# Fantom-foundation/go-txflow

Measured on AMD Instinct MI355X. Metric: verified+tallied TxVotes/sec, higher is better.
Workload: dtype u32

## Files before the change

go-txflow_amd/csrc/ed25519_dev.h:

```cpp
#pragma once
#include "fe.h"
#include "sc.h"
#include "sha2.h"
#include "ge.h"

namespace txv {

template <int W>
struct Tab {
  static constexpr int kPositions = (256 + W - 1) / W;
  static constexpr int kEntries = (1 << (W - 1)) + 1;
  static constexpr bool kLongTop = false;
  static constexpr int kTopEntries = kEntries;
  static constexpr size_t kWords = (size_t)kPositions * kEntries * kEntryWords;
  static constexpr uint64_t kBuildLanes = (uint64_t)kPositions * ((kEntries - 1) / 8);
};

template <>
struct Tab<21> {
  static constexpr int kPositions = 12;
  static constexpr int kEntries = (1 << 20) + 1;
  static constexpr bool kLongTop = true;
  static constexpr int kTopEntries = (1 << 21) + 9;
  static constexpr size_t kWords = ((size_t)(kPositions - 1) * kEntries + kTopEntries) * kEntryWords;
// ... 53 lines not shown
  const uint32_t pad_word = total >> 3, pad_shift = 56u - 8u * (total & 7u);
  const uint32_t last = 16u * nblk - 1u;
  uint64_t nx[16];
#pragma unroll
  for (int t = 0; t < 16; ++t) nx[t] = t < pre_words ? pre[t] : msg_word(m, (uint32_t)(t - pre_words));
  for (uint32_t b = 0; b < nblk; ++b) {
    uint64_t w[16];
#pragma unroll
    for (int t = 0; t < 16; ++t) {
      const uint32_t gw = 16u * b + (uint32_t)t;
      uint64_t v = nx[t];
      if (gw == pad_word) v |= 0x80ull << pad_shift;
      if (gw == last) v = (uint64_t)total * 8u;
      w[t] = v;
    }
    if (b + 1 < nblk) {
#pragma unroll
      for (int t = 0; t < 16; ++t) nx[t] = msg_word(m, 16u * (b + 1) + (uint32_t)t - (uint32_t)pre_words);
    }
    sha512_block(st, w);
  }
#pragma unroll
  for (int k = 0; k < 8; ++k) {
    digest_le[2 * k] = bswap32((uint32_t)(st[k] >> 32));
    digest_le[2 * k + 1] = bswap32((uint32_t)st[k]);
  }
}

TXV_HD void sha512_prefixed2(uint32_t dig0[16], const uint64_t* pre0, const MsgView& m0, uint32_t dig1[16],
                             const uint64_t* pre1, const MsgView& m1, int pre_words) {
  uint64_t st0[8], st1[8];
  sha512_init(st0);
  sha512_init(st1);
  const uint32_t tot0 = 8u * (uint32_t)pre_words + m0.len, tot1 = 8u * (uint32_t)pre_words + m1.len;
  const uint32_t nb0 = sha512_nblocks(tot0), nb1 = sha512_nblocks(tot1), nb = nb0 > nb1 ? nb0 : nb1;
  const uint32_t pw0 = tot0 >> 3, ps0 = 56u - 8u * (tot0 & 7u), last0 = 16u * nb0 - 1u;
  const uint32_t pw1 = tot1 >> 3, ps1 = 56u - 8u * (tot1 & 7u), last1 = 16u * nb1 - 1u;
  for (uint32_t b = 0; b < nb; ++b) {
    uint64_t w0[16], w1[16];
#pragma unroll
    for (int t = 0; t < 16; ++t) {
      const uint32_t gw = 16u * b + (uint32_t)t;
      uint64_t v0 = (b == 0 && t < pre_words) ? pre0[t] : msg_word(m0, gw - (uint32_t)pre_words);
      uint64_t v1 = (b == 0 && t < pre_words) ? pre1[t] : msg_word(m1, gw - (uint32_t)pre_words);
      if (gw == pw0) v0 |= 0x80ull << ps0;
      if (gw == last0) v0 = (uint64_t)tot0 * 8u;
      if (gw == pw1) v1 |= 0x80ull << ps1;
      if (gw == last1) v1 = (uint64_t)tot1 * 8u;
      w0[t] = v0;
      w1[t] = v1;
    }
    uint64_t s0[8], s1[8];
#pragma unroll
    for (int k = 0; k < 8; ++k) { s0[k] = st0[k]; s1[k] = st1[k]; }
    sha512_block2(s0, w0, s1, w1);
#pragma unroll
    for (int k = 0; k < 8; ++k) {
      if (b < nb0) st0[k] = s0[k];
      if (b < nb1) st1[k] = s1[k];
    }
  }
#pragma unroll
  for (int k = 0; k < 8; ++k) {
    dig0[2 * k] = bswap32((uint32_t)(st0[k] >> 32));
    dig0[2 * k + 1] = bswap32((uint32_t)st0[k]);
    dig1[2 * k] = bswap32((uint32_t)(st1[k] >> 32));
    dig1[2 * k + 1] = bswap32((uint32_t)st1[k]);
  }
}

template <int W, typename Ptr>
TXV_HD void load_entry_w(Ptr tab, int pos, int idx, bool neg, fe10& qp, fe10& qm, fe10& qd) {
#if defined(TXV_EXP_L2_TABLES)
  const size_t base = (size_t)(1 + (idx & 1)) * kEntryWords;
#else
  const size_t base = (size_t)(uint32_t)(pos * Tab<W>::kEntries + idx) * kEntryWords;
#endif
#ifndef TXV_ENTRY_LOADS
#define TXV_ENTRY_LOADS 1
#endif
#if TXV_ENTRY_LOADS == 2
  const uint4* e4 = reinterpret_cast<const uint4*>(&tab[base]);
  uint32_t w[32];
#pragma unroll
  for (int j = 0; j < 8; ++j) {
    const uint4 x = e4[j];
    w[4 * j] = x.x; w[4 * j + 1] = x.y; w[4 * j + 2] = x.z; w[4 * j + 3] = x.w;
  }
#pragma unroll
  for (int i = 0; i < 10; ++i) {
    qd.v[i] = w[kEntryQd + i];
    qm.v[i] = neg ? w[i] : w[kEntryQm + i];
    qp.v[i] = neg ? w[kEntryQm + i] : w[i];
  }
#else
  const uint32_t op = neg ? kEntryQm : 0u, om = neg ? 0u : kEntryQm;
  const uint2* d2 = reinterpret_cast<const uint2*>(&tab[base + kEntryQd]);
  const uint2 d0 = d2[0];
  const uint4 d1 = reinterpret_cast<const uint4*>(d2 + 1)[0], d3 = reinterpret_cast<const uint4*>(d2 + 1)[1];
  const uint4* m4 = reinterpret_cast<const uint4*>(&tab[base + om]);
  const uint4 m0 = m4[0], m1 = m4[1];
  const uint2 m2 = reinterpret_cast<const uint2*>(m4 + 2)[0];
  const uint4* p4 = reinterpret_cast<const uint4*>(&tab[base + op]);
  const uint4 p0 = p4[0], p1 = p4[1];
  const uint2 p2 = reinterpret_cast<const uint2*>(p4 + 2)[0];
  qp.v[0] = p0.x; qp.v[1] = p0.y; qp.v[2] = p0.z; qp.v[3] = p0.w;
  qp.v[4] = p1.x; qp.v[5] = p1.y; qp.v[6] = p1.z; qp.v[7] = p1.w; qp.v[8] = p2.x; qp.v[9] = p2.y;
  qm.v[0] = m0.x; qm.v[1] = m0.y; qm.v[2] = m0.z; qm.v[3] = m0.w;
  qm.v[4] = m1.x; qm.v[5] = m1.y; qm.v[6] = m1.z; qm.v[7] = m1.w; qm.v[8] = m2.x; qm.v[9] = m2.y;
  qd.v[0] = d0.x; qd.v[1] = d0.y; qd.v[2] = d1.x; qd.v[3] = d1.y;
  qd.v[4] = d1.z; qd.v[5] = d1.w; qd.v[6] = d3.x; qd.v[7] = d3.y; qd.v[8] = d3.z; qd.v[9] = d3.w;
#endif
}

template <int W>
TXV_HD int next_digit(uint32_t s[8], uint32_t& carry) {
  constexpr uint32_t mask = (1u << W) - 1u, half = 1u << (W - 1);
  const uint32_t d = (s[0] & mask) + carry;
  carry = (d + half) >> W;
#pragma unroll
  for (int i = 0; i < 7; ++i) s[i] = (s[i] >> W) | (s[i + 1] << (32 - W));
  s[7] >>= W;
  return (int)d - (int)(carry << W);
}

template <int W>
TXV_HD int table_digit(uint32_t s[8], uint32_t& carry, int pos) {
  if constexpr (Tab<W>::kLongTop) {
    if (pos == Tab<W>::kPositions - 1) return (int)(s[0] + carry);
  }
  return next_digit<W>(s, carry);
}

template <int W, int N>
TXV_HD void signed_digits(const uint32_t s[8], int d[N]) {
  constexpr uint32_t mask = (1u << W) - 1u, half = 1u << (W - 1);
  uint32_t carry = 0;
#pragma unroll
  for (int i = 0; i < N; ++i) {
    const int b = W * i, w = b >> 5, o = b & 31;
    uint32_t win = s[w] >> o;
    if (o + W > 32 && w + 1 < 8) win |= s[w + 1] << (32 - o);
    if (Tab<W>::kLongTop && i == Tab<W>::kPositions - 1) {
      static_assert(!Tab<W>::kLongTop || W * (Tab<W>::kPositions - 1) % 32 + 22 <= 32, "top digit in one word");
      d[i] = (int)(win + carry);
      break;
    }
    const uint32_t dd = (win & mask) + carry;
    carry = (dd + half) >> W;
    d[i] = (int)dd - (int)(carry << W);
  }
}

template <int WB, int WA, typename PtrB, typename PtrA>
TXV_HD ge_ext double_scalarmult_w2(PtrB tb, PtrA ta, const uint32_t s_in[8], const uint32_t k_in[8], bool use_a) {
  static_assert(WB >= WA, "B window must be at least the A window");
  uint32_t s[8], k[8], cs = 0, ck = 0;
#pragma unroll
  for (int i = 0; i < 8; ++i) { s[i] = s_in[i]; k[i] = k_in[i]; }
  fe10 qp, qm, qd;
  ge10_ext P;
  {
    const int ds = next_digit<WB>(s, cs);
    load_entry_w<WB>(tb, 0, ds < 0 ? -ds : ds, ds < 0, qp, qm, qd);
    P = ge10_from_entry(qp, qm);
  }
  for (int pos = 0; pos < Tab<WA>::kPositions; ++pos) {
    if (pos > 0 && pos < Tab<WB>::kPositions) {
      const int ds = next_digit<WB>(s, cs);
      load_entry_w<WB>(tb, pos, ds < 0 ? -ds : ds, ds < 0, qp, qm, qd);
      P = ge10_madd(P, qp, qm, qd, ds < 0);
    }
    if (use_a) {
      const int dk = table_digit<WA>(k, ck, pos);
      load_entry_w<WA>(ta, pos, dk < 0 ? -dk : dk, dk > 0, qp, qm, qd);
      P = ge10_madd(P, qp, qm, qd, dk > 0);
    }
  }
  ge_ext R;
  R.X = fe_from_fe10(P.X);
  R.Y = fe_from_fe10(P.Y);
  R.Z = fe_from_fe10(P.Z);
  R.T = fe_zero();
  return R;
}
template <int W, typename PtrB, typename PtrA>
TXV_HD ge_ext double_scalarmult_w(PtrB tb, PtrA ta, const uint32_t s_in[8], const uint32_t k_in[8], bool use_a) {
  return double_scalarmult_w2<W, W>(tb, ta, s_in, k_in, use_a);
}

template <typename PtrB, typename PtrA>
TXV_HD ge_ext double_scalarmult_fixed(PtrB tb, PtrA ta, const uint32_t s[8], const uint32_t k[8], bool use_a) {
  return double_scalarmult_w<4>(tb, ta, s, k, use_a);
}

TXV_HD ge_ext ge_mul_small(const ge_ext& P, uint32_t m) {
  ge_ext R = P;
  int top = 31 - __builtin_clz(m);
  for (int b = top - 1; b >= 0; --b) {
    R = ge_dbl(R);
    if ((m >> b) & 1u) R = ge_add(R, P);
  }
  return R;
}

TXV_HD void base_point_words(uint32_t w[8]) {
  const uint32_t b[8] = {0x66666658u, 0x66666666u, 0x66666666u, 0x66666666u,
                         0x66666666u, 0x66666666u, 0x66666666u, 0x66666666u};
#pragma unroll
  for (int i = 0; i < 8; ++i) w[i] = b[i];
}

}
```

go-txflow_amd/csrc/fe10.h:

```cpp
#pragma once
#include "fe.h"

namespace txv {

struct fe10 { uint32_t v[10]; };

#define TXV_W10(i) (((i) & 1) ? 25 : 26)
#define TXV_M10(i) (((i) & 1) ? 0x1ffffffu : 0x3ffffffu)

TXV_HD uint32_t fe10_2p(int i) { return i == 0 ? 0x7ffffdau : ((i & 1) ? 0x3fffffeu : 0x7fffffeu); }

TXV_HD fe10 fe10_zero() { fe10 r; for (int i = 0; i < 10; ++i) r.v[i] = 0; return r; }
TXV_HD fe10 fe10_one() { fe10 r = fe10_zero(); r.v[0] = 1; return r; }

TXV_HD fe10 fe10_add(const fe10& a, const fe10& b) {
  fe10 r;
#pragma unroll
  for (int i = 0; i < 10; ++i) r.v[i] = a.v[i] + b.v[i];
  return r;
}
TXV_HD fe10 fe10_sub(const fe10& a, const fe10& b) {
  fe10 r;
#pragma unroll
  for (int i = 0; i < 10; ++i) r.v[i] = (a.v[i] + fe10_2p(i)) - b.v[i];
  return r;
}
TXV_HD fe10 fe10_cneg(const fe10& a, bool neg) {
  const uint32_t m = neg ? 0xffffffffu : 0u;
  fe10 r;
#pragma unroll
  for (int i = 0; i < 10; ++i) r.v[i] = (a.v[i] ^ m) + (m & (fe10_2p(i) + 1u));
  return r;
}

TXV_HD fe10 fe10_carry(const fe10& a) {
  fe10 r = a;
  uint32_t c = 0;
#pragma unroll
  for (int i = 0; i < 10; ++i) {
    const uint32_t t = r.v[i] + c;
    c = t >> TXV_W10(i);
    r.v[i] = t & TXV_M10(i);
  }
  const uint32_t t = r.v[0] + 19u * c;
  r.v[0] = t & 0x3ffffffu;
  r.v[1] += t >> 26;
  return r;
}

#ifndef TXV_FE10_MUL
#define TXV_FE10_MUL 1
#endif
TXV_HD uint64_t fe10_col(uint64_t cin, const uint32_t a[10], const uint32_t b[10]) {
#if defined(__HIP_DEVICE_COMPILE__) && TXV_FE10_MUL == 2
  uint64_t x, y, cc;
  asm("v_mad_u64_u32 %0, %2, %3, %13, %23\n\t"
      "v_mad_u64_u32 %1, %2, %4, %14, 0\n\t"
      "v_mad_u64_u32 %0, %2, %5, %15, %0\n\t"
      "v_mad_u64_u32 %1, %2, %6, %16, %1\n\t"
      "v_mad_u64_u32 %0, %2, %7, %17, %0\n\t"
      "v_mad_u64_u32 %1, %2, %8, %18, %1\n\t"
      "v_mad_u64_u32 %0, %2, %9, %19, %0\n\t"
      "v_mad_u64_u32 %1, %2, %10, %20, %1\n\t"
      "v_mad_u64_u32 %0, %2, %11, %21, %0\n\t"
      "v_mad_u64_u32 %1, %2, %12, %22, %1\n\t"
      "v_lshl_add_u64 %0, %0, 0, %1"
      : "=&v"(x), "=&v"(y), "=&s"(cc)
      : "v"(a[0]), "v"(a[1]), "v"(a[2]), "v"(a[3]), "v"(a[4]), "v"(a[5]), "v"(a[6]), "v"(a[7]), "v"(a[8]), "v"(a[9]),
        "v"(b[0]), "v"(b[1]), "v"(b[2]), "v"(b[3]), "v"(b[4]), "v"(b[5]), "v"(b[6]), "v"(b[7]), "v"(b[8]), "v"(b[9]),
        "v"(cin));
  return x;
#elif defined(__HIP_DEVICE_COMPILE__) && TXV_FE10_MUL == 1
  uint64_t acc, cc;
  asm("v_mad_u64_u32 %0, %1, %2, %12, %22\n\t"
      "v_mad_u64_u32 %0, %1, %3, %13, %0\n\t"
      "v_mad_u64_u32 %0, %1, %4, %14, %0\n\t"
      "v_mad_u64_u32 %0, %1, %5, %15, %0\n\t"
      "v_mad_u64_u32 %0, %1, %6, %16, %0\n\t"
      "v_mad_u64_u32 %0, %1, %7, %17, %0\n\t"
      "v_mad_u64_u32 %0, %1, %8, %18, %0\n\t"
      "v_mad_u64_u32 %0, %1, %9, %19, %0\n\t"
      "v_mad_u64_u32 %0, %1, %10, %20, %0\n\t"
      "v_mad_u64_u32 %0, %1, %11, %21, %0"
      : "=&v"(acc), "=&s"(cc)
      : "v"(a[0]), "v"(a[1]), "v"(a[2]), "v"(a[3]), "v"(a[4]), "v"(a[5]), "v"(a[6]), "v"(a[7]), "v"(a[8]), "v"(a[9]),
        "v"(b[0]), "v"(b[1]), "v"(b[2]), "v"(b[3]), "v"(b[4]), "v"(b[5]), "v"(b[6]), "v"(b[7]), "v"(b[8]), "v"(b[9]),
        "v"(cin));
  return acc;
#else
  uint64_t acc = cin;
  for (int i = 0; i < 10; ++i) acc += (uint64_t)a[i] * b[i];
  return acc;
#endif
}

TXV_HD fe10 fe10_mul(const fe10& f, const fe10& g) {
  uint32_t g19[10], f2[10];
#pragma unroll
  for (int j = 1; j < 10; ++j) g19[j] = 19u * g.v[j];
#pragma unroll
  for (int i = 0; i < 10; ++i) f2[i] = (i & 1) ? f.v[i] + f.v[i] : f.v[i];
  g19[0] = 0;
  fe10 h;
  uint64_t acc = 0;
#pragma unroll
  for (int k = 0; k < 10; ++k) {
    uint32_t a[10], b[10];
#pragma unroll
    for (int i = 0; i < 10; ++i) {
      a[i] = ((i & 1) && !(k & 1)) ? f2[i] : f.v[i];
      b[i] = i <= k ? g.v[k - i] : g19[k + 10 - i];
    }
    acc = fe10_col(acc, a, b);
    h.v[k] = (uint32_t)acc & TXV_M10(k);
    acc >>= TXV_W10(k);
  }
  const uint64_t t = (uint64_t)(uint32_t)acc * 19u + h.v[0] + ((uint64_t)((uint32_t)(acc >> 32) * 19u) << 32);
  h.v[0] = (uint32_t)t & 0x3ffffffu;
  h.v[1] += (uint32_t)(t >> 26);
  return h;
}

TXV_HD void fe10_col2(uint64_t c1, const uint32_t a[10], const uint32_t b[10], uint64_t c2, const uint32_t x[10],
                      const uint32_t y[10], uint64_t& o1, uint64_t& o2) {
#if defined(__HIP_DEVICE_COMPILE__)
  uint64_t p, q, cc;
  asm("v_mad_u64_u32 %0, %2, %3, %13, %43\n\t"
      "v_mad_u64_u32 %1, %2, %23, %33, %44\n\t"
      "v_mad_u64_u32 %0, %2, %4, %14, %0\n\t"
      "v_mad_u64_u32 %1, %2, %24, %34, %1\n\t"
      "v_mad_u64_u32 %0, %2, %5, %15, %0\n\t"
      "v_mad_u64_u32 %1, %2, %25, %35, %1\n\t"
      "v_mad_u64_u32 %0, %2, %6, %16, %0\n\t"
      "v_mad_u64_u32 %1, %2, %26, %36, %1\n\t"
      "v_mad_u64_u32 %0, %2, %7, %17, %0\n\t"
      "v_mad_u64_u32 %1, %2, %27, %37, %1\n\t"
      "v_mad_u64_u32 %0, %2, %8, %18, %0\n\t"
      "v_mad_u64_u32 %1, %2, %28, %38, %1\n\t"
      "v_mad_u64_u32 %0, %2, %9, %19, %0\n\t"
      "v_mad_u64_u32 %1, %2, %29, %39, %1\n\t"
      "v_mad_u64_u32 %0, %2, %10, %20, %0\n\t"
      "v_mad_u64_u32 %1, %2, %30, %40, %1\n\t"
      "v_mad_u64_u32 %0, %2, %11, %21, %0\n\t"
      "v_mad_u64_u32 %1, %2, %31, %41, %1\n\t"
      "v_mad_u64_u32 %0, %2, %12, %22, %0\n\t"
      "v_mad_u64_u32 %1, %2, %32, %42, %1"
      : "=&v"(p), "=&v"(q), "=&s"(cc)
      : "v"(a[0]), "v"(a[1]), "v"(a[2]), "v"(a[3]), "v"(a[4]), "v"(a[5]), "v"(a[6]), "v"(a[7]), "v"(a[8]), "v"(a[9]),
        "v"(b[0]), "v"(b[1]), "v"(b[2]), "v"(b[3]), "v"(b[4]), "v"(b[5]), "v"(b[6]), "v"(b[7]), "v"(b[8]), "v"(b[9]),
        "v"(x[0]), "v"(x[1]), "v"(x[2]), "v"(x[3]), "v"(x[4]), "v"(x[5]), "v"(x[6]), "v"(x[7]), "v"(x[8]), "v"(x[9]),
        "v"(y[0]), "v"(y[1]), "v"(y[2]), "v"(y[3]), "v"(y[4]), "v"(y[5]), "v"(y[6]), "v"(y[7]), "v"(y[8]), "v"(y[9]),
        "v"(c1), "v"(c2));
  o1 = p;
  o2 = q;
#else
  uint64_t p = c1, q = c2;
  for (int i = 0; i < 10; ++i) {
    p += (uint64_t)a[i] * b[i];
    q += (uint64_t)x[i] * y[i];
  }
  o1 = p;
  o2 = q;
#endif
}

TXV_HD void fe10_mul2(const fe10& f1, const fe10& g1, const fe10& f2, const fe10& g2, fe10& h1, fe10& h2) {
  uint32_t g19a[10], f2a[10], g19b[10], f2b[10];
#pragma unroll
  for (int j = 1; j < 10; ++j) {
    g19a[j] = 19u * g1.v[j];
    g19b[j] = 19u * g2.v[j];
  }
#pragma unroll
  for (int i = 0; i < 10; ++i) {
    f2a[i] = (i & 1) ? f1.v[i] + f1.v[i] : f1.v[i];
    f2b[i] = (i & 1) ? f2.v[i] + f2.v[i] : f2.v[i];
  }
  g19a[0] = g19b[0] = 0;
  fe10 r1, r2;
  uint64_t acc1 = 0, acc2 = 0;
#pragma unroll
  for (int k = 0; k < 10; ++k) {
    uint32_t a[10], b[10], x[10], y[10];
#pragma unroll
    for (int i = 0; i < 10; ++i) {
      const bool dbl = (i & 1) && !(k & 1);
      a[i] = dbl ? f2a[i] : f1.v[i];
      x[i] = dbl ? f2b[i] : f2.v[i];
      b[i] = i <= k ? g1.v[k - i] : g19a[k + 10 - i];
      y[i] = i <= k ? g2.v[k - i] : g19b[k + 10 - i];
    }
    fe10_col2(acc1, a, b, acc2, x, y, acc1, acc2);
    r1.v[k] = (uint32_t)acc1 & TXV_M10(k);
    r2.v[k] = (uint32_t)acc2 & TXV_M10(k);
    acc1 >>= TXV_W10(k);
    acc2 >>= TXV_W10(k);
  }
  const uint64_t t1 = (uint64_t)(uint32_t)acc1 * 19u + r1.v[0] + ((uint64_t)((uint32_t)(acc1 >> 32) * 19u) << 32);
  const uint64_t t2 = (uint64_t)(uint32_t)acc2 * 19u + r2.v[0] + ((uint64_t)((uint32_t)(acc2 >> 32) * 19u) << 32);
  r1.v[0] = (uint32_t)t1 & 0x3ffffffu;
  r1.v[1] += (uint32_t)(t1 >> 26);
  r2.v[0] = (uint32_t)t2 & 0x3ffffffu;
  r2.v[1] += (uint32_t)(t2 >> 26);
  h1 = r1;
  h2 = r2;
}

TXV_HD fe10 fe10_strict(const fe10& a) {
  fe10 r = fe10_carry(a);
  uint32_t c = 0;
#pragma unroll
  for (int i = 1; i < 10; ++i) {
    const uint32_t t = r.v[i] + c;
    c = t >> TXV_W10(i);
    r.v[i] = t & TXV_M10(i);
  }
  const uint32_t t = r.v[0] + 19u * c;
  r.v[0] = t & 0x3ffffffu;
  r.v[1] += t >> 26;
  return r;
}

TXV_HD fe10 fe10_from_fe(const fe& a) {
  fe10 r;
  const uint32_t top = a.v[7] >> 31;
  int bit = 0;
#pragma unroll
  for (int i = 0; i < 10; ++i) {
    const int w = bit >> 5, s = bit & 31;
    uint32_t x = a.v[w] >> s;
    if (s + TXV_W10(i) > 32 && w < 7) x |= a.v[w + 1] << (32 - s);
    r.v[i] = x & TXV_M10(i);
    bit += TXV_W10(i);
  }
  r.v[0] += 19u * top;
  return r;
}

TXV_HD fe fe_from_fe10(const fe10& a) {
  const fe10 s = fe10_strict(a);
  fe r;
#pragma unroll
  for (int w = 0; w < 8; ++w) r.v[w] = 0;
  int bit = 0;
#pragma unroll
  for (int i = 0; i < 10; ++i) {
    const int w = bit >> 5, sh = bit & 31;
    r.v[w] |= s.v[i] << sh;
    if (sh + TXV_W10(i) > 32 && w < 7) r.v[w + 1] |= s.v[i] >> (32 - sh);
    bit += TXV_W10(i);
  }
  return r;
}

}
```

go-txflow_amd/csrc/kernels_verify.hip:

```cpp
#include <algorithm>
#include <cstdlib>

#include "ed25519_dev.h"
#include "fe_inv_var.h"
#include "txv_device.h"

using namespace txv;

#ifndef TXV_K1A_PREFETCH
#define TXV_K1A_PREFETCH 0
#endif

#ifndef TXV_INV_VAR
#define TXV_INV_VAR 1
#endif
__device__ __forceinline__ fe verify_invert(const fe& z) {
#if TXV_INV_VAR
  return fe_invert_var(z);
#else
  return fe_invert(z);
#endif
}

template <int W>
// ... 204 lines not shown
    }
    if (!act[0] && !act[1]) continue;
    ge_ext R;
    for (int h = 0; h < 2; ++h) {
      const uint32_t i = vi[h];
      if (act[h]) {
        const uint32_t v = a.val[i];
        uint32_t s[8], k[8];
#pragma unroll
        for (int j = 0; j < 8; ++j) { s[j] = a.sig[(size_t)(8 + j) * a.n_pad + i]; k[j] = a.kbuf[(size_t)j * a.n_pad + i]; }
        R = double_scalarmult_w<W>(a.btable, a.atables + (size_t)tab_slot(a, v) * Tab<W>::kWords, s, k, true);
      } else {
        R = ge_identity();
      }
      if (h == 0) {
#pragma unroll
        for (int j = 0; j < 8; ++j) {
          park[j][threadIdx.x] = R.X.v[j];
          park[8 + j][threadIdx.x] = R.Y.v[j];
          park[16 + j][threadIdx.x] = R.Z.v[j];
        }
      }
    }
    fe X0, Y0, Z0;
#pragma unroll
    for (int j = 0; j < 8; ++j) {
      X0.v[j] = park[j][threadIdx.x];
      Y0.v[j] = park[8 + j][threadIdx.x];
      Z0.v[j] = park[16 + j][threadIdx.x];
    }
    const fe inv = verify_invert(fe_mul(Z0, R.Z));
    uint32_t enc[8];
#pragma unroll
    for (int h = 0; h < 2; ++h) {
      if (h == 0) ge_encode_zinv(enc, X0, Y0, fe_mul(inv, R.Z));
      else ge_encode_zinv(enc, R.X, R.Y, fe_mul(inv, Z0));
      if (act[h]) {
        uint32_t diff = 0;
#pragma unroll
        for (int j = 0; j < 8; ++j) diff |= enc[j] ^ a.sig[(size_t)j * a.n_pad + vi[h]];
        a.ok_out[vi[h]] = diff == 0;
      }
    }
  }
}

#ifndef TXV_K1B_PREFETCH
#define TXV_K1B_PREFETCH 1
#endif

#ifndef TXV_K1B_NO_GATHER
#define TXV_K1B_NO_GATHER 0
#endif
__device__ __forceinline__ void entries_to_lds(const uint32_t* base, uint32_t e_l, uint4* buf) {
  if (TXV_K1B_NO_GATHER) return;
  const int lane = threadIdx.x & 63;
  uint32_t e[8];
#pragma unroll
  for (int i = 0; i < 8; ++i) e[i] = (uint32_t)__builtin_amdgcn_ds_bpermute((8 * i + (lane >> 3)) << 2, (int)e_l);
  TXV_SCHED_FENCE();
#pragma unroll
  for (int i = 0; i < 8; ++i) {
    const uint32_t piece = (uint32_t)((lane & 7) + 8 * i + (lane >> 3)) & 7u;
    const uint32_t* g = base + (size_t)e[i] * kEntryWords + piece * 4u;
    __builtin_amdgcn_global_load_lds((const __attribute__((address_space(1))) void*)g,
                                     (__attribute__((address_space(3))) void*)(buf + 64 * i), 16, 0, 0);
  }
}

__device__ __forceinline__ const uint4* entry_piece(const uint4* buf, int j) {
  const int e = threadIdx.x & 63;
  return buf + 64 * (e >> 3) + 8 * (e & 7) + ((j - e) & 7);
}

__device__ __forceinline__ fe10 entry_field_lds(const uint4* buf, bool neg, int role) {
  fe10 r;
  if (role == 2) {
    const uint2 d0 = reinterpret_cast<const uint2*>(entry_piece(buf, 5))[1];
    const uint4 d1 = *entry_piece(buf, 6), d2 = *entry_piece(buf, 7);
    r.v[0] = d0.x; r.v[1] = d0.y; r.v[2] = d1.x; r.v[3] = d1.y;
    r.v[4] = d1.z; r.v[5] = d1.w; r.v[6] = d2.x; r.v[7] = d2.y; r.v[8] = d2.z; r.v[9] = d2.w;
    return r;
  }
  const int j0 = (neg != (role == 1)) ? 3 : 0;
  const uint4 p0 = *entry_piece(buf, j0), p1 = *entry_piece(buf, j0 + 1);
  const uint2 p2 = *reinterpret_cast<const uint2*>(entry_piece(buf, j0 + 2));
  r.v[0] = p0.x; r.v[1] = p0.y; r.v[2] = p0.z; r.v[3] = p0.w;
  r.v[4] = p1.x; r.v[5] = p1.y; r.v[6] = p1.z; r.v[7] = p1.w; r.v[8] = p2.x; r.v[9] = p2.y;
  return r;
}

template <int WB, int WA, int PD>
__device__ __forceinline__ ge_ext double_scalarmult_pf(const uint32_t* tb, const uint32_t* ta, uint32_t va,
                                                       const uint32_t s_in[8], const uint32_t k_in[8], uint4* buf) {
  static_assert(WB >= WA, "B window must be at least the A window");
  static_assert(PD == 1 || PD == 2, "prefetch depth");
  constexpr int nB = Tab<WB>::kPositions, nA = Tab<WA>::kPositions, nT = nB + nA;
  uint32_t s[8], k[8], cs = 0, ck = 0;
#pragma unroll
  for (int i = 0; i < 8; ++i) { s[i] = s_in[i]; k[i] = k_in[i]; }
  auto issue = [&](int t) -> bool {
    const bool isB = t < 2 * nB && !(t & 1);
    const int pos = t < 2 * nB ? (t >> 1) : t - nB;
    uint4* b = buf + (PD == 2 ? (t & 1) * 512 : 0);
    if (isB) {
      const int d = next_digit<WB>(s, cs);
      entries_to_lds(tb, (uint32_t)(pos * Tab<WB>::kEntries + (d < 0 ? -d : d)), b);
      return d < 0;
    }
    const int d = table_digit<WA>(k, ck, pos);
    entries_to_lds(ta, (uint32_t)(va * (uint32_t)(Tab<WA>::kWords / kEntryWords) + pos * Tab<WA>::kEntries + (d < 0 ? -d : d)), b);
    return d > 0;
  };
  ge10_ext P;
  bool neg = issue(0), neg2 = false;
  if (PD == 2) neg2 = issue(1);
#pragma unroll 1
  for (int t = 0; t < nT - 1; ++t) {
    if (PD == 2 && t + 1 < nT) asm volatile("s_waitcnt vmcnt(8)" ::: "memory");
    else asm volatile("s_waitcnt vmcnt(0)" ::: "memory");
    const bool neg_t = neg;
    const uint4* bt = buf + (PD == 2 ? (t & 1) * 512 : 0);
    auto next = [&]() {
      asm volatile("s_waitcnt lgkmcnt(0)" ::: "memory");
      if (PD == 2) {
        neg = neg2;
        if (t + 2 < nT) neg2 = issue(t + 2);
      } else if (t + 1 < nT) {
        neg = issue(t + 1);
      }
    };
    if (t) {
      P = ge10_madd_rd(P, [&](int role) { return entry_field_lds(bt, neg_t, role); }, neg_t, next);
    } else {
      const fe10 qp = entry_field_lds(bt, neg_t, 0), qm = entry_field_lds(bt, neg_t, 1);
      next();
      P = ge10_from_entry(qp, qm);
    }
  }
  {
    asm volatile("s_waitcnt vmcnt(0)" ::: "memory");
    const uint4* bt = buf + (PD == 2 ? ((nT - 1) & 1) * 512 : 0);
    const bool neg_t = neg;
    P = ge10_madd_rd<false>(P, [&](int role) { return entry_field_lds(bt, neg_t, role); }, neg_t, [] {});
  }
  ge_ext R;
  R.X = fe_from_fe10(P.X);
  R.Y = fe_from_fe10(P.Y);
  R.Z = fe_from_fe10(P.Z);
  R.T = fe_zero();
  return R;
}

template <int WB, int WA>
__device__ __forceinline__ ge_ext double_scalarmult_rs(const uint32_t* tb, const uint32_t* ta, uint32_t va,
                                                       const uint32_t s_in[8], const uint32_t k_in[8], uint4* buf) {
  static_assert(WB >= WA, "B window must be at least the A window");
  constexpr int nB = Tab<WB>::kPositions, nA = Tab<WA>::kPositions, nT = nB + nA;
  static_assert(nT >= 4, "schedule too short");
  uint32_t s[8], k[8], cs = 0, ck = 0;
#pragma unroll
  for (int i = 0; i < 8; ++i) { s[i] = s_in[i]; k[i] = k_in[i]; }
  auto issue = [&](int t) -> bool {
    const bool isB = t < 2 * nB && !(t & 1);
    const int pos = t < 2 * nB ? (t >> 1) : t - nB;
    uint4* b = buf + (t & 1) * 512;
    if (isB) {
      const int d = next_digit<WB>(s, cs);
      entries_to_lds(tb, (uint32_t)(pos * Tab<WB>::kEntries + (d < 0 ? -d : d)), b);
      return d < 0;
    }
    const int d = table_digit<WA>(k, ck, pos);
    entries_to_lds(ta, (uint32_t)(va * (uint32_t)(Tab<WA>::kWords / kEntryWords) + pos * Tab<WA>::kEntries + (d < 0 ? -d : d)), b);
    return d > 0;
  };
  const bool n0 = issue(0), n1a = issue(1);
  asm volatile("s_waitcnt vmcnt(8)" ::: "memory");
  fe10 qp = entry_field_lds(buf, n0, 0), qm = entry_field_lds(buf, n0, 1), qd;
  asm volatile("s_waitcnt lgkmcnt(0)" ::: "memory");
  bool nq2 = issue(2);
  ge10_ext P = ge10_from_entry(qp, qm);
  TXV_SCHED_FENCE();
  asm volatile("s_waitcnt vmcnt(8)" ::: "memory");
  qp = entry_field_lds(buf + 512, n1a, 0);
  qm = entry_field_lds(buf + 512, n1a, 1);
  qd = entry_field_lds(buf + 512, n1a, 2);
  asm volatile("s_waitcnt lgkmcnt(0)" ::: "memory");
  bool ncur = n1a, nq1 = nq2;
  nq2 = issue(3);
  TXV_SCHED_FENCE();
#pragma unroll 1
  for (int t = 1; t < nT; ++t) {
    const bool more = t + 1 < nT;
    const fe10 C = fe10_cneg(fe10_mul(P.T, qd), ncur);
    TXV_SCHED_FENCE();
    const fe10 A = fe10_mul(fe10_sub(P.Y, P.X), qm);
    TXV_SCHED_FENCE();
    const fe10 B = fe10_mul(fe10_add(P.Y, P.X), qp);
    TXV_SCHED_FENCE();
    if (more) {
      if (t + 2 < nT) asm volatile("s_waitcnt vmcnt(8)" ::: "memory");
      else asm volatile("s_waitcnt vmcnt(0)" ::: "memory");
      const uint4* bn = buf + ((t + 1) & 1) * 512;
      qp = entry_field_lds(bn, nq1, 0);
      qm = entry_field_lds(bn, nq1, 1);
      qd = entry_field_lds(bn, nq1, 2);
    }
    TXV_SCHED_FENCE();
    const fe10 E = fe10_sub(B, A), H = fe10_add(B, A);
    const fe10 G = fe10_add(P.Z, C), F = fe10_sub(P.Z, C);
    ge10_ext r;
    r.X = fe10_mul(F, E);
    TXV_SCHED_FENCE();
    if (more) {
      asm volatile("s_waitcnt lgkmcnt(0)" ::: "memory");
      ncur = nq1;
      nq1 = nq2;
      if (t + 3 < nT) nq2 = issue(t + 3);
    }
    TXV_SCHED_FENCE();
    r.Y = fe10_mul(H, G);
    TXV_SCHED_FENCE();
    r.Z = fe10_mul(F, G);
    TXV_SCHED_FENCE();
    r.T = more ? fe10_mul(H, E) : fe10_zero();
    TXV_SCHED_FENCE();
    P = r;
  }
  ge_ext R;
  R.X = fe_from_fe10(P.X);
  R.Y = fe_from_fe10(P.Y);
  R.Z = fe_from_fe10(P.Z);
  R.T = fe_zero();
  return R;
}

#ifndef TXV_K1B_REGSTAGE
#define TXV_K1B_REGSTAGE 1
#endif
template <int WB, int WA, int PD>
__device__ __forceinline__ ge_ext k1b_walk(const uint32_t* tb, const uint32_t* ta, uint32_t va, const uint32_t s[8],
                                           const uint32_t k[8], uint4* buf) {
  if constexpr (TXV_K1B_REGSTAGE && PD == 2) return double_scalarmult_rs<WB, WA>(tb, ta, va, s, k, buf);
  else return double_scalarmult_pf<WB, WA, PD>(tb, ta, va, s, k, buf);
}

#ifndef TXV_PARK_LAST
#define TXV_PARK_LAST 1
#endif
#ifndef TXV_V4_WAVES
#define TXV_V4_WAVES 2
#endif
#ifndef TXV_EXP_NO_TAIL
#define TXV_EXP_NO_TAIL 0
#endif
#ifndef TXV_EXP_NO_WALK
#define TXV_EXP_NO_WALK 0
#endif
#ifdef TXV_K1B_VGPRS
#define TXV_K1B_VGPR_ATTR __attribute__((amdgpu_num_vgpr(TXV_K1B_VGPRS)))
#else
#define TXV_K1B_VGPR_ATTR
#endif
template <int BLOCK, int WB, int WA, int V>
__global__ void __launch_bounds__(BLOCK, V == 8 ? 2 : TXV_V4_WAVES * BLOCK / 512) TXV_K1B_VGPR_ATTR txv_k_scalarmult_multi(VerifyArgs a) {
  const uint32_t n_grp = (a.n_work + 64u * V - 1u) / (64u * V) * 64u;
  const uint32_t groups = gridDim.x >= 8 ? 8u : 1u;
  const uint32_t grp = blockIdx.x % groups, blocks_in_grp = gridDim.x / groups + (grp < gridDim.x % groups);
  const uint32_t chunk = ((n_grp + groups - 1) / groups + 63u) & ~63u;
  const uint32_t lo = grp * chunk, hi = min(n_grp, lo + chunk);
  const uint32_t stride = blocks_in_grp * BLOCK;
  const uint32_t gwave = (blockIdx.x * BLOCK + threadIdx.x) >> 6;
  uint32_t* park = a.park + (size_t)gwave * (V - 1 + TXV_PARK_LAST) * TXV_PARK_WORDS * 64 + (threadIdx.x & 63);
#if TXV_K1B_PREFETCH
  constexpr int PD = V == 8 ? 2 : 1;
  __shared__ uint4 pf[BLOCK / 64][PD * 8 * 64];
  uint4* wbuf = pf[__builtin_amdgcn_readfirstlane(threadIdx.x >> 6)];
#endif
  for (uint32_t g = lo + (blockIdx.x / groups) * BLOCK + threadIdx.x; g < hi; g += stride) {
    uint32_t act = 0;
#pragma unroll
    for (int h = 0; h < V; ++h) {
      const uint32_t idx = (g & ~63u) * V + 64u * h + (g & 63u);
      if (idx < a.n_work && a.ok_out[a.order ? a.order[idx] : idx] == 2) act |= 1u << h;
    }
#if TXV_K1B_PREFETCH
    if (__builtin_amdgcn_ballot_w64(act != 0) == 0) continue;
#else
    if (!act) continue;
#endif
    ge_ext R;
    fe P;
#pragma unroll 1
    for (int h = 0; h < V; ++h) {
#if TXV_K1B_PREFETCH
      {
        const bool on = act >> h & 1u;
        const uint32_t idx = (g & ~63u) * V + 64u * h + (g & 63u);
        const uint32_t i = on ? (a.order ? a.order[idx] : idx) : 0u;
        uint32_t s[8], k[8];
#pragma unroll
        for (int j = 0; j < 8; ++j) {
          s[j] = on ? a.sig[(size_t)(8 + j) * a.n_pad + i] : 0u;
          k[j] = on ? a.kbuf[(size_t)j * a.n_pad + i] : 0u;
        }
#if TXV_EXP_NO_WALK
        (void)wbuf;
#pragma unroll
        for (int j = 0; j < 8; ++j) { R.X.v[j] = s[j] | 1u; R.Y.v[j] = k[j] | 2u; R.Z.v[j] = s[j] ^ k[j] ^ 5u; R.T.v[j] = 0; }
#else
        R = k1b_walk<WB, WA, PD>(a.btable, a.atables, on ? tab_slot(a, a.val[i]) : 0u, s, k, wbuf);
#endif
      }
#else
      if (act >> h & 1u) {
        const uint32_t idx = (g & ~63u) * V + 64u * h + (g & 63u);
        const uint32_t i = a.order ? a.order[idx] : idx;
        uint32_t s[8], k[8];
#pragma unroll
        for (int j = 0; j < 8; ++j) { s[j] = a.sig[(size_t)(8 + j) * a.n_pad + i]; k[j] = a.kbuf[(size_t)j * a.n_pad + i]; }
        R = double_scalarmult_w2<WB, WA>(a.btable, a.atables + (size_t)tab_slot(a, a.val[i]) * Tab<WA>::kWords, s, k, true);
      } else {
        R = ge_identity();
      }
#endif
      P = h ? fe_mul(P, R.Z) : R.Z;
      if (h < V - 1 || TXV_PARK_LAST) {
        uint32_t* slot = park + h * TXV_PARK_WORDS * 64;
#pragma unroll
        for (int j = 0; j < 8; ++j) {
          slot[j * 64] = R.X.v[j];
          slot[(8 + j) * 64] = R.Y.v[j];
          slot[(16 + j) * 64] = P.v[j];
          slot[(24 + j) * 64] = R.Z.v[j];
        }
      }
    }
#if TXV_EXP_NO_TAIL
    if (act & 1u) a.ok_out[(g & ~63u) * V + (g & 63u)] = P.v[0] == 0x12345u;
    continue;
#endif
    fe inv = verify_invert(P);
#pragma unroll 1
    for (int h = V - 1; h >= 0; --h) {
      fe X, Y, Z, zi;
      if (h == V - 1 && !TXV_PARK_LAST) {
        X = R.X; Y = R.Y; Z = R.Z;
      } else {
        const uint32_t* slot = park + h * TXV_PARK_WORDS * 64;
#pragma unroll
        for (int j = 0; j < 8; ++j) {
          X.v[j] = slot[j * 64];
          Y.v[j] = slot[(8 + j) * 64];
          Z.v[j] = slot[(24 + j) * 64];
        }
      }
      if (h) {
        const uint32_t* prev = park + (h - 1) * TXV_PARK_WORDS * 64;
        fe Pp;
#pragma unroll
        for (int j = 0; j < 8; ++j) Pp.v[j] = prev[(16 + j) * 64];
        zi = fe_mul(inv, Pp);
        inv = fe_mul(inv, Z);
      } else {
        zi = inv;
      }
      if (act >> h & 1u) {
        const uint32_t idx = (g & ~63u) * V + 64u * h + (g & 63u);
        const uint32_t i = a.order ? a.order[idx] : idx;
        uint32_t enc[8];
        ge_encode_zinv(enc, X, Y, zi);
        uint32_t diff = 0;
#pragma unroll
        for (int j = 0; j < 8; ++j) diff |= enc[j] ^ a.sig[(size_t)j * a.n_pad + i];
        a.ok_out[i] = diff == 0;
      }
    }
  }
}

#ifndef TXV_K1B_DYNAMIC
// ... 718 lines not shown
```

Measured before the change: 770.5 million.

## Factor LDS-staged scalar walk into reusable pingpong template with scalar mask constants

```diff
diff --git a/go-txflow_amd/csrc/ed25519_dev.h b/go-txflow_amd/csrc/ed25519_dev.h
--- a/go-txflow_amd/csrc/ed25519_dev.h
+++ b/go-txflow_amd/csrc/ed25519_dev.h
@@ -229,6 +229,112 @@
   }
 }
 
+#ifndef TXV_K1B_PINGPONG
+#define TXV_K1B_PINGPONG 0
+#endif
+template <int N> struct walk_int { static constexpr int value = N; };
+template <int WB, int WA, class Mem, int nB = Tab<WB>::kPositions, int nA = Tab<WA>::kPositions,
+          bool kPair = TXV_K1B_PINGPONG != 0>
+TXV_HD ge10_ext walk_pingpong(Mem& m, const uint32_t s_in[8], const uint32_t k_in[8]) {
+  static_assert(WB >= WA && nB <= nA && nB >= 2, "B window must be at least the A window");
+  constexpr int nT = nB + nA;
+  static_assert(nT >= 4, "schedule too short");
+  [[maybe_unused]] constexpr int kTopPos = Tab<WA>::kPositions - 1;
+  uint32_t s[8], k[8], cs = 0, ck = 0;
+#pragma unroll
+  for (int i = 0; i < 8; ++i) { s[i] = s_in[i]; k[i] = k_in[i]; }
+  auto issue_b = [&](int b, int pos) -> bool {
+    const int d = next_digit<WB>(s, cs);
+    m.digit(true, pos, d);
+    m.template gather<true>(b, (uint32_t)(pos * Tab<WB>::kEntries + (d < 0 ? -d : d)));
+    return d < 0;
+  };
+  auto issue_a = [&](auto top, int b, int pos) -> bool {
+    int d;
+    if constexpr (!Tab<WA>::kLongTop || decltype(top)::value == 0) d = next_digit<WA>(k, ck);
+    else d = table_digit<WA>(k, ck, pos);
+    m.digit(false, pos, d);
+    m.template gather<false>(b, (uint32_t)(pos * Tab<WA>::kEntries + (d < 0 ? -d : d)));
+    return d > 0;
+  };
+  auto issue_t = [&](int t) -> bool {
+    const bool isB = t < 2 * nB && !(t & 1);
+    const int pos = t < 2 * nB ? (t >> 1) : t - nB;
+    return isB ? issue_b(t & 1, pos) : issue_a(walk_int<2>(), t & 1, pos);
+  };
+  fe10 qp, qm, qd;
+  bool ncur, nq1, nq2;
+  auto add = [&](const ge10_ext& P, int bn, bool more, bool more2, auto nxt) -> ge10_ext {
+    const fe10 C = fe10_cneg(fe10_mul(P.T, qd), ncur);
+    TXV_SCHED_FENCE();
+    const fe10 A = fe10_mul(fe10_sub(P.Y, P.X), qm);
+    TXV_SCHED_FENCE();
+    const fe10 B = fe10_mul(fe10_add(P.Y, P.X), qp);
+    TXV_SCHED_FENCE();
+    if (more) {
+      m.landed(more2);
+      m.read(bn, nq1, qp, qm, &qd);
+    }
+    TXV_SCHED_FENCE();
+    const fe10 E = fe10_sub(B, A), H = fe10_add(B, A);
+    const fe10 G = fe10_add(P.Z, C), F = fe10_sub(P.Z, C);
+    ge10_ext r;
+    r.X = fe10_mul(F, E);
+    TXV_SCHED_FENCE();
+    if (more) {
+      m.read_done();
+      ncur = nq1;
+      nq1 = nq2;
+      nxt();
+    }
+    TXV_SCHED_FENCE();
+    r.Y = fe10_mul(H, G);
+    TXV_SCHED_FENCE();
+    r.Z = fe10_mul(F, G);
+    TXV_SCHED_FENCE();
+    r.T = more ? fe10_mul(H, E) : fe10_zero();
+    TXV_SCHED_FENCE();
+    return r;
+  };
+  const bool n0 = issue_t(0), n1a = issue_t(1);
+  m.landed(true);
+  m.read(0, n0, qp, qm, nullptr);
+  m.read_done();
+  nq2 = issue_t(2);
+  ge10_ext P = ge10_from_entry(qp, qm);
+  TXV_SCHED_FENCE();
+  m.landed(true);
+  m.read(1, n1a, qp, qm, &qd);
+  m.read_done();
+  ncur = n1a;
+  nq1 = nq2;
+  nq2 = issue_t(3);
+  TXV_SCHED_FENCE();
+  int t = 1;
+  if constexpr (kPair) {
+    constexpr int kTopPair = Tab<WA>::kLongTop && nB - 1 >= kTopPos ? 2 : 0;
+#pragma unroll 1
+    for (; t + 4 < 2 * nB; t += 2) {
+      const ge10_ext Q = add(P, 0, true, true, [&] { nq2 = issue_b(0, (t + 3) >> 1); });
+      P = add(Q, 1, true, true, [&] { nq2 = issue_a(walk_int<kTopPair>(), 1, (t + 4) >> 1); });
+    }
+#pragma unroll 1
+    for (; t < nT; ++t) {
+      P = add(P, (t + 1) & 1, t + 1 < nT, t + 2 < nT, [&] {
+        if (t + 3 < nT) nq2 = issue_a(walk_int<2>(), (t + 3) & 1, t + 3 - nB);
+      });
+    }
+  } else {
+#pragma unroll 1
+    for (; t < nT; ++t) {
+      P = add(P, (t + 1) & 1, t + 1 < nT, t + 2 < nT, [&] {
+        if (t + 3 < nT) nq2 = issue_t(t + 3);
+      });
+    }
+  }
+  return P;
+}
+
 template <int WB, int WA, typename PtrB, typename PtrA>
 TXV_HD ge_ext double_scalarmult_w2(PtrB tb, PtrA ta, const uint32_t s_in[8], const uint32_t k_in[8], bool use_a) {
   static_assert(WB >= WA, "B window must be at least the A window");
diff --git a/go-txflow_amd/csrc/fe10.h b/go-txflow_amd/csrc/fe10.h
--- a/go-txflow_amd/csrc/fe10.h
+++ b/go-txflow_amd/csrc/fe10.h
@@ -8,7 +8,28 @@
 #define TXV_W10(i) (((i) & 1) ? 25 : 26)
 #define TXV_M10(i) (((i) & 1) ? 0x1ffffffu : 0x3ffffffu)
 
-TXV_HD uint32_t fe10_2p(int i) { return i == 0 ? 0x7ffffdau : ((i & 1) ? 0x3fffffeu : 0x7fffffeu); }
+#ifndef TXV_FE10_SCONST
+#define TXV_FE10_SCONST 1
+#endif
+TXV_HD uint32_t fe10_sconst(uint32_t c) {
+#if defined(__HIP_DEVICE_COMPILE__) && TXV_FE10_SCONST
+  uint32_t r;
+  asm("s_mov_b32 %0, %1" : "=s"(r) : "i"(c));
+  return r;
+#else
+  return c;
+#endif
+}
+TXV_HD uint32_t fe10_mask(int i) { return fe10_sconst(TXV_M10(i)); }
+
+TXV_HD uint32_t fe10_2p(int i) {
+  const uint32_t c = i == 0 ? 0x7ffffdau : ((i & 1) ? 0x3fffffeu : 0x7fffffeu);
+#if TXV_FE10_SCONST >= 2
+  return fe10_sconst(c);
+#else
+  return c;
+#endif
+}
 
 TXV_HD fe10 fe10_zero() { fe10 r; for (int i = 0; i < 10; ++i) r.v[i] = 0; return r; }
 TXV_HD fe10 fe10_one() { fe10 r = fe10_zero(); r.v[0] = 1; return r; }
@@ -112,11 +133,11 @@
       b[i] = i <= k ? g.v[k - i] : g19[k + 10 - i];
     }
     acc = fe10_col(acc, a, b);
-    h.v[k] = (uint32_t)acc & TXV_M10(k);
+    h.v[k] = (uint32_t)acc & fe10_mask(k);
     acc >>= TXV_W10(k);
   }
   const uint64_t t = (uint64_t)(uint32_t)acc * 19u + h.v[0] + ((uint64_t)((uint32_t)(acc >> 32) * 19u) << 32);
-  h.v[0] = (uint32_t)t & 0x3ffffffu;
+  h.v[0] = (uint32_t)t & fe10_mask(0);
   h.v[1] += (uint32_t)(t >> 26);
   return h;
 }
diff --git a/go-txflow_amd/csrc/kernels_verify.hip b/go-txflow_amd/csrc/kernels_verify.hip
--- a/go-txflow_amd/csrc/kernels_verify.hip
+++ b/go-txflow_amd/csrc/kernels_verify.hip
@@ -380,81 +380,74 @@
   return R;
 }
 
+__device__ __forceinline__ const uint32_t* entry_addr(uint64_t base, uint32_t e) {
+  uint64_t r, cc;
+  asm("v_mad_u64_u32 %0, %1, %2, %3, %4" : "=&v"(r), "=&s"(cc) : "v"(e), "s"((uint32_t)(kEntryWords * 4)), "v"(base));
+  return reinterpret_cast<const uint32_t*>(r);
+}
+
+struct WalkLds {
+  uint4* buf;
+  uint64_t gb, ga;
+  uint32_t ea;
+  int lane, perm;
+
+  __device__ __forceinline__ WalkLds(const uint32_t* tb, const uint32_t* ta, uint32_t entries_a, uint32_t va, uint4* b)
+      : buf(b), lane(threadIdx.x & 63) {
+    const uint32_t piece = (uint32_t)((lane & 7) + (lane >> 3)) & 7u;
+    gb = (uint64_t)(tb + piece * 4u);
+    ga = (uint64_t)(ta + piece * 4u);
+    ea = va * entries_a;
+    perm = (lane >> 3) << 2;
+  }
+  __device__ __forceinline__ void digit(bool, int, int) {}
+  template <bool B>
+  __device__ __forceinline__ void gather(int b, uint32_t e) {
+    if (TXV_K1B_NO_GATHER) return;
+    const uint32_t e_l = B ? e : ea + e;
+    uint32_t x[8];
+    int src = perm;
+    asm volatile("" : "+v"(src));
+#pragma unroll
+    for (int i = 0; i < 8; ++i) x[i] = (uint32_t)__builtin_amdgcn_ds_bpermute(src + 32 * i, (int)e_l);
+    TXV_SCHED_FENCE();
+#pragma unroll
+    for (int i = 0; i < 8; ++i) {
+      __builtin_amdgcn_global_load_lds((const __attribute__((address_space(1))) void*)entry_addr(B ? gb : ga, x[i]),
+                                       (__attribute__((address_space(3))) void*)(buf + 512 * b + 64 * i), 16, 0, 0);
+    }
+  }
+  __device__ __forceinline__ void landed(bool keep) {
+    if (keep) asm volatile("s_waitcnt vmcnt(8)" ::: "memory");
+    else asm volatile("s_waitcnt vmcnt(0)" ::: "memory");
+  }
+  __device__ __forceinline__ void read(int b, bool neg, fe10& qp, fe10& qm, fe10* qd) {
+    const uint4* bt = buf + 512 * b;
+    const uint4 *lo[3], *hi[3];
+#pragma unroll
+    for (int j = 0; j < 3; ++j) { lo[j] = entry_piece(bt, j); hi[j] = entry_piece(bt, 3 + j); }
+    {
+      const uint4 p0 = *(neg ? hi[0] : lo[0]), p1 = *(neg ? hi[1] : lo[1]);
+      const uint2 p2 = *reinterpret_cast<const uint2*>(neg ? hi[2] : lo[2]);
+      qp.v[0] = p0.x; qp.v[1] = p0.y; qp.v[2] = p0.z; qp.v[3] = p0.w;
+      qp.v[4] = p1.x; qp.v[5] = p1.y; qp.v[6] = p1.z; qp.v[7] = p1.w; qp.v[8] = p2.x; qp.v[9] = p2.y;
+    }
+    {
+      const uint4 p0 = *(neg ? lo[0] : hi[0]), p1 = *(neg ? lo[1] : hi[1]);
+      const uint2 p2 = *reinterpret_cast<const uint2*>(neg ? lo[2] : hi[2]);
+      qm.v[0] = p0.x; qm.v[1] = p0.y; qm.v[2] = p0.z; qm.v[3] = p0.w;
+      qm.v[4] = p1.x; qm.v[5] = p1.y; qm.v[6] = p1.z; qm.v[7] = p1.w; qm.v[8] = p2.x; qm.v[9] = p2.y;
+    }
+    if (qd) *qd = entry_field_lds(bt, neg, 2);
+  }
+  __device__ __forceinline__ void read_done() { asm volatile("s_waitcnt lgkmcnt(0)" ::: "memory"); }
+};
+
 template <int WB, int WA>
 __device__ __forceinline__ ge_ext double_scalarmult_rs(const uint32_t* tb, const uint32_t* ta, uint32_t va,
                                                        const uint32_t s_in[8], const uint32_t k_in[8], uint4* buf) {
-  static_assert(WB >= WA, "B window must be at least the A window");
-  constexpr int nB = Tab<WB>::kPositions, nA = Tab<WA>::kPositions, nT = nB + nA;
-  static_assert(nT >= 4, "schedule too short");
-  uint32_t s[8], k[8], cs = 0, ck = 0;
-#pragma unroll
-  for (int i = 0; i < 8; ++i) { s[i] = s_in[i]; k[i] = k_in[i]; }
-  auto issue = [&](int t) -> bool {
-    const bool isB = t < 2 * nB && !(t & 1);
-    const int pos = t < 2 * nB ? (t >> 1) : t - nB;
-    uint4* b = buf + (t & 1) * 512;
-    if (isB) {
-      const int d = next_digit<WB>(s, cs);
-      entries_to_lds(tb, (uint32_t)(pos * Tab<WB>::kEntries + (d < 0 ? -d : d)), b);
-      return d < 0;
-    }
-    const int d = table_digit<WA>(k, ck, pos);
-    entries_to_lds(ta, (uint32_t)(va * (uint32_t)(Tab<WA>::kWords / kEntryWords) + pos * Tab<WA>::kEntries + (d < 0 ? -d : d)), b);
-    return d > 0;
-  };
-  const bool n0 = issue(0), n1a = issue(1);
-  asm volatile("s_waitcnt vmcnt(8)" ::: "memory");
-  fe10 qp = entry_field_lds(buf, n0, 0), qm = entry_field_lds(buf, n0, 1), qd;
-  asm volatile("s_waitcnt lgkmcnt(0)" ::: "memory");
-  bool nq2 = issue(2);
-  ge10_ext P = ge10_from_entry(qp, qm);
-  TXV_SCHED_FENCE();
-  asm volatile("s_waitcnt vmcnt(8)" ::: "memory");
-  qp = entry_field_lds(buf + 512, n1a, 0);
-  qm = entry_field_lds(buf + 512, n1a, 1);
-  qd = entry_field_lds(buf + 512, n1a, 2);
-  asm volatile("s_waitcnt lgkmcnt(0)" ::: "memory");
-  bool ncur = n1a, nq1 = nq2;
-  nq2 = issue(3);
-  TXV_SCHED_FENCE();
-#pragma unroll 1
-  for (int t = 1; t < nT; ++t) {
-    const bool more = t + 1 < nT;
-    const fe10 C = fe10_cneg(fe10_mul(P.T, qd), ncur);
-    TXV_SCHED_FENCE();
-    const fe10 A = fe10_mul(fe10_sub(P.Y, P.X), qm);
-    TXV_SCHED_FENCE();
-    const fe10 B = fe10_mul(fe10_add(P.Y, P.X), qp);
-    TXV_SCHED_FENCE();
-    if (more) {
-      if (t + 2 < nT) asm volatile("s_waitcnt vmcnt(8)" ::: "memory");
-      else asm volatile("s_waitcnt vmcnt(0)" ::: "memory");
-      const uint4* bn = buf + ((t + 1) & 1) * 512;
-      qp = entry_field_lds(bn, nq1, 0);
-      qm = entry_field_lds(bn, nq1, 1);
-      qd = entry_field_lds(bn, nq1, 2);
-    }
-    TXV_SCHED_FENCE();
-    const fe10 E = fe10_sub(B, A), H = fe10_add(B, A);
-    const fe10 G = fe10_add(P.Z, C), F = fe10_sub(P.Z, C);
-    ge10_ext r;
-    r.X = fe10_mul(F, E);
-    TXV_SCHED_FENCE();
-    if (more) {
-      asm volatile("s_waitcnt lgkmcnt(0)" ::: "memory");
-      ncur = nq1;
-      nq1 = nq2;
-      if (t + 3 < nT) nq2 = issue(t + 3);
-    }
-    TXV_SCHED_FENCE();
-    r.Y = fe10_mul(H, G);
-    TXV_SCHED_FENCE();
-    r.Z = fe10_mul(F, G);
-    TXV_SCHED_FENCE();
-    r.T = more ? fe10_mul(H, E) : fe10_zero();
-    TXV_SCHED_FENCE();
-    P = r;
-  }
+  WalkLds m(tb, ta, (uint32_t)(Tab<WA>::kWords / kEntryWords), va, buf);
+  const ge10_ext P = walk_pingpong<WB, WA>(m, s_in, k_in);
   ge_ext R;
   R.X = fe_from_fe10(P.X);
   R.Y = fe_from_fe10(P.Y);
```

Result: no change. 774.9 million (median of 6 runs) (+0.6%).
